# turboderp-org/exllamav2

Measured on NVIDIA H100. Metric: decode tokens/sec (bs=1) Llama2-7B EXL2-4.0bpw, higher is better.
Workload: dtype fp16 (int2-8 weights, fp32 accumulate)

## Files before the change

exllamav2_b200/csrc/attn_q4.cu:

```cuda
#include <algorithm>
#include <map>
#include <mutex>

#include "gemv_i8.cuh"
#include "kv_format.cuh"
#include "qmatrix.cuh"

namespace exl2b {

extern unsigned long long* g_dbg;
extern int g_dbg_cta, g_dbg_slot;

constexpr int AQ_THREADS = 256;
constexpr int AQ_WARPS = 8;
constexpr int AQ_MAX_QLEN = 8;

struct AttnQ4Params {
    const half* q;
    const half* k_new;
    const half* v_new;
    uint8_t* k_q;
    half* k_s;
    uint8_t* v_q;
    half* v_s;
    const int32_t* cache_seqlens;
    const int32_t* block_table;
    half* out;
    half* out_xp;
    const uint16_t* out_invperm;
    int q_len, H, KVH, hd, page_size, pages_per_seq, max_ctx;
    float scale_log2;
    const half* rope_sin;
    const half* rope_cos;
    int rope_neox, sincos_size;
    int out_plain;
    int32_t* err;
    int sc_len;
    int stage;
    int ring_slots;
    int batch;
    int busy_ctas;
    unsigned int* slot_cnt;
    int nsplit;
    float* ws;
    unsigned int* cnt;
    unsigned long long* dbg;
    int dbg_cta;
    int pass_len;
};
constexpr int AQ_SPLIT_MIN = 512;
constexpr int AQ_SUB = 128;
constexpr int AQ_RING = 4;
constexpr int AQ_STAGE = 512;
constexpr int AQ_SMEM_MAX = 200 * 1024;
constexpr int AQ_PASS_SMEM = 114 * 1024;
constexpr int AQ_PASS_MIN = 512;
constexpr int AQ_PASS_ALIGN = 256;
constexpr int AQ_QPAD = 36;
constexpr int AQ_QIB = 80;

__host__ __device__ constexpr int aq_sub(int kb, int vb) { return AQ_SUB * 4 / (kb > vb ? kb : vb); }

struct AttnSmem {
    uint32_t qrot, qi, qsum, qscl, red, wred, new_q, new_s, new_y, pages, sc, kst, vst, ksst, vsst, rq, rs, total;
};
__host__ __device__ inline AttnSmem attn_smem_map(int hd, int kb, int vb, int pages_per_seq, int sc_len, int stage, bool ring) {
    const uint32_t nsc = hd / 32, rowk = hd * kb / 8, rowv = hd * vb / 8, sub = aq_sub(kb, vb);
    AttnSmem m;
    m.qrot = 0;
    m.qi = m.qrot + nsc * AQ_QPAD * 4;
    m.qsum = m.qi + nsc * AQ_QIB;
    m.qscl = m.qsum + nsc * 4;
    m.red = m.qscl + nsc * 4;
    m.wred = m.red + AQ_WARPS * hd * 4;
    m.new_q = m.wred + 2 * AQ_WARPS * 4;
    m.new_s = m.new_q + AQ_MAX_QLEN * (rowk + rowv);
    m.new_y = m.new_s + 2 * AQ_MAX_QLEN * nsc * 2;
    m.pages = m.new_y + 2 * AQ_MAX_QLEN * hd * 4;
    m.sc = m.pages + ((pages_per_seq + 3) & ~3) * 4;
    m.kst = m.sc + ((sc_len + 3) & ~3) * 4;
    m.vst = m.kst + stage * rowk;
    m.ksst = m.vst + stage * rowv;
    m.vsst = m.ksst + stage * nsc * 2;
    m.rq = m.vsst + stage * nsc * 2;
    m.rs = m.rq + AQ_RING * sub * (rowk > rowv ? rowk : rowv);
    m.total = ring ? m.rs + AQ_RING * sub * nsc * 2 : m.rq;
    return m;
}

template <bool GLOBAL, typename T>
__device__ __forceinline__ T ld_rows(const T* p) {
    if constexpr (GLOBAL) return __ldg(p);
    else return *p;
}

template <int HD>
__device__ __forceinline__ half2 load_roped(const half* __restrict__ row, int un, int lane, const AttnQ4Params& P, int pos) {
    const half2 v = reinterpret_cast<const half2*>(row + un * 64)[lane];
    if (!P.rope_sin) return v;
    const half* sr = P.rope_sin + (size_t)pos * P.sincos_size;
    const half* cr = P.rope_cos + (size_t)pos * P.sincos_size;
    if (P.rope_neox) {
        half2 o;
        int col;
        bool first;
        if constexpr (HD == 128) {
            o = reinterpret_cast<const half2*>(row + (un ^ 1) * 64)[lane];
            col = 2 * lane;
            first = (un == 0);
        } else {
            o = __shfl_xor_sync(0xffffffffu, v, 16);
            col = 2 * (lane & 15);
            first = lane < 16;
        }
        const half2 c2 = *reinterpret_cast<const half2*>(cr + col);
        const half2 s2 = *reinterpret_cast<const half2*>(sr + col);
        if (first) return __hfma2(v, c2, __hmul2(o, __hneg2(s2)));
        return __hfma2(v, c2, __hmul2(o, s2));
    }
    const int col = un * 64 + 2 * lane;
    const half2 c01 = *reinterpret_cast<const half2*>(cr + col);
    half2 s01 = *reinterpret_cast<const half2*>(sr + col);
    uint32_t sb = *reinterpret_cast<uint32_t*>(&s01) ^ (1u << 15);
    s01 = *reinterpret_cast<half2*>(&sb);
    return __hfma2(__lowhigh2highlow(v), s01, __hmul2(v, c01));
}

__device__ __forceinline__ float nib_f(uint32_t n) { return __uint_as_float(0x4B000000u | n) - 8388616.0f; }
__device__ __forceinline__ float byte_f(uint32_t n) { return __uint_as_float(0x4B000000u | n) - 8388736.0f; }

__device__ __forceinline__ void cta_exit(const AttnQ4Params& P) {
    if (threadIdx.x == 0) slot_release(P.slot_cnt);
}

template <int HD, int KB, int VB>
struct AttnCta {
    static_assert((KB == 4 || KB == 8) && (VB == 4 || VB == 8), "element widths are 4 or 8 bits");
    static constexpr int ROWBK = HD * KB / 8;
    static constexpr int ROWBV = HD * VB / 8;
    static constexpr int ROWB = ROWBK > ROWBV ? ROWBK : ROWBV;
    static constexpr int SUB = aq_sub(KB, VB);
    static constexpr int NSC = HD / 32;
    static constexpr int VEC = HD / 32;
    static constexpr int UNITS = HD / 64;
    static constexpr int TPR = NSC, RPP = AQ_THREADS / TPR;
    static constexpr int KW = KB / 4;
    static constexpr uint32_t KFILL = KB == 4 ? 0x88888888u : 0x80808080u;

    const AttnQ4Params& P;
    float* qrot;
    uint8_t* qi;
    int* qsum;
    float* qscl;
    float* red;
    float* wred;
    uint8_t* new_q;
    half* new_s;
    float* new_y;
    int* pages_s;
    float* sc;
    uint8_t *kst, *vst;
    half *ksst, *vsst;
    uint8_t* rq;
    half* rs;
    int h, b, z, tid, warp, lane, group, kvh, kblk, krow;
    int seqlen, ns_act, p_lo, p_hi, c_hi, n_st, ntail;
    const int* bt;

    __device__ __forceinline__ AttnCta(const AttnQ4Params& P_, uint8_t* smem) : P(P_) {
        const AttnSmem m = attn_smem_map(HD, KB, VB, P.pages_per_seq, P.sc_len, P.stage, true);
        qrot = reinterpret_cast<float*>(smem + m.qrot);
        qi = smem + m.qi;
        qsum = reinterpret_cast<int*>(smem + m.qsum);
        qscl = reinterpret_cast<float*>(smem + m.qscl);
        red = reinterpret_cast<float*>(smem + m.red);
        wred = reinterpret_cast<float*>(smem + m.wred);
        new_q = smem + m.new_q;
        new_s = reinterpret_cast<half*>(smem + m.new_s);
        new_y = reinterpret_cast<float*>(smem + m.new_y);
        pages_s = reinterpret_cast<int*>(smem + m.pages);
        sc = reinterpret_cast<float*>(smem + m.sc);
        kst = smem + m.kst;
        vst = smem + m.vst;
        ksst = reinterpret_cast<half*>(smem + m.ksst);
        vsst = reinterpret_cast<half*>(smem + m.vsst);
        rq = smem + m.rq;
        rs = reinterpret_cast<half*>(smem + m.rs);
        h = (int)blockIdx.x % P.H;
        b = ((int)blockIdx.x / P.H) % P.batch;
        z = (int)blockIdx.x / (P.H * P.batch);
        tid = threadIdx.x;
        warp = tid >> 5;
        lane = tid & 31;
        group = P.H / P.KVH;
        kvh = h / group;
        kblk = tid & (TPR - 1);
        krow = tid / TPR;
    }

    __device__ __forceinline__ size_t row(int p) const {
        const int page = bt[p / P.page_size];
        return ((size_t)page * P.page_size + p % P.page_size) * P.KVH + kvh;
    }

    __device__ __forceinline__ bool prologue() {
        seqlen = P.cache_seqlens[b];
        if (seqlen < 0 || seqlen + P.q_len > P.max_ctx) {
            if (tid == 0 && P.err) atomicOr(P.err, 1);
            return false;
        }
        bt = P.block_table + (size_t)b * P.pages_per_seq;
        ns_act = 1;
        p_lo = 0;
        p_hi = seqlen + P.q_len;
        if (P.nsplit > 1) {
            const int n_all = seqlen + 1;
            ns_act = min(P.nsplit, max(1, (n_all + AQ_SPLIT_MIN - 1) / AQ_SPLIT_MIN));
            if (z >= ns_act) return false;
            const int chunk = (n_all + ns_act - 1) / ns_act;
            p_lo = z * chunk;
            p_hi = min(n_all, p_lo + chunk);
        }
        c_hi = min(p_hi, seqlen);
        n_st = max(0, min(c_hi - p_lo, P.stage));
        constexpr int CHK = ROWBK / 16, CHV = ROWBV / 16, CH = CHK > CHV ? CHK : CHV;
        for (int idx = tid; idx < n_st * CH; idx += AQ_THREADS) {
            const int pos = idx / CH, ch = idx - pos * CH;
            const size_t r = row(p_lo + pos);
            if (ch < CHK) cp_async16(smem_addr(kst + pos * ROWBK + ch * 16), P.k_q + r * ROWBK + ch * 16);
            if (ch < CHV) cp_async16(smem_addr(vst + pos * ROWBV + ch * 16), P.v_q + r * ROWBV + ch * 16);
        }
        for (int pos = tid; pos < n_st; pos += AQ_THREADS) {
            const size_t r = row(p_lo + pos);
            cp_async_small<NSC * 2>(smem_addr(ksst + pos * NSC), P.k_s + r * NSC);
            cp_async_small<NSC * 2>(smem_addr(vsst + pos * NSC), P.v_s + r * NSC);
        }
        asm volatile("cp.async.commit_group;" ::: "memory");
        for (int i = tid; i < P.pages_per_seq; i += AQ_THREADS) pages_s[i] = bt[i];
        bt = pages_s;
        ntail = ring_chunks();
        return true;
    }
    __device__ __forceinline__ int ring_chunks() const {
        return (P.ring_slots && c_hi > p_lo + n_st) ? (c_hi - (p_lo + n_st) + SUB - 1) / SUB : 0;
    }

    __device__ __forceinline__ void begin_pass(int lo, int hi, int nst) {
        p_lo = lo;
        c_hi = min(hi, seqlen);
        n_st = nst;
        ntail = ring_chunks();
    }

    __device__ __forceinline__ void rotate_q(int i, int un) {
        const half2 qh = load_roped<HD>(P.q + (((size_t)b * P.q_len + i) * P.H + h) * HD, un, lane, P, seqlen + i);
        float2 w = hadamard32_f(__half22float2(qh), lane);
        const float f = P.scale_log2 * (1.0f / 32.0f);
        const int e = un * 64 + 2 * lane;
        w.x *= f;
        w.y *= f;
        qrot[(e >> 5) * AQ_QPAD + (e & 31)] = w.x;
        qrot[(e >> 5) * AQ_QPAD + (e & 31) + 1] = w.y;
        float amax = fmaxf(fabsf(w.x), fabsf(w.y));
#pragma unroll
        for (int o = 1; o < 16; o <<= 1) amax = fmaxf(amax, __shfl_xor_sync(0xffffffffu, amax, o));
        const uint32_t ef = (__float_as_uint(amax * 1.000030518f) >> 23) & 0xffu;
        const float inv = amax > 0.f ? __uint_as_float((268u - ef) << 23) : 0.f;
        const uint32_t q0 = __float_as_uint(fmaf(w.x, inv, 12582912.f)), q1 = __float_as_uint(fmaf(w.y, inv, 12582912.f));
        int sum = (int)(q0 + q1 - 2u * 0x4B400000u);
#pragma unroll
        for (int o = 1; o < 16; o <<= 1) sum += __shfl_xor_sync(0xffffffffu, sum, o);
        const int blk = e >> 5, l16 = lane & 15;
        if constexpr (KB == 4) {
            const int j = l16 >> 2, m = l16 & 3;
            uint8_t* qb = qi + blk * AQ_QIB + j * 16 + m;
            qb[0] = (uint8_t)(q0 >> 8);
            qb[4] = (uint8_t)q0;
            qb[8] = (uint8_t)(q1 >> 8);
            qb[12] = (uint8_t)q1;
        } else {
            const int w8 = l16 >> 1;
            uint8_t* qb = qi + blk * AQ_QIB + (w8 >> 1) * 16 + (w8 & 1) * 8 + (l16 & 1) * 2;
            qb[0] = (uint8_t)(q0 >> 8);
            qb[1] = (uint8_t)(q1 >> 8);
            qb[4] = (uint8_t)q0;
            qb[5] = (uint8_t)q1;
        }
        if (l16 == 0) {
            qsum[blk] = sum;
            qscl[blk] = amax > 0.f ? __uint_as_float((ef - 14u) << 23) : 0.f;
        }
    }

    __device__ __forceinline__ void new_rows_and_first_query() {
        if (warp >= AQ_WARPS - UNITS) rotate_q(0, warp - (AQ_WARPS - UNITS));
        const int n_jobs = 2 * P.q_len * UNITS;
        for (int job = (warp >= AQ_WARPS - UNITS && n_jobs <= AQ_WARPS - UNITS) ? n_jobs : warp; job < n_jobs; job += AQ_WARPS) {
            const int kv = job / (P.q_len * UNITS), r = job - kv * P.q_len * UNITS;
            const int i = r / UNITS, un = r - i * UNITS;
            const half* src = (kv ? P.v_new : P.k_new) + (((size_t)b * P.q_len + i) * P.KVH + kvh) * HD;
            half2 w2 = kv ? reinterpret_cast<const half2*>(src + un * 64)[lane] : load_roped<HD>(src, un, lane, P, seqlen + i);
            {
                const float2 y = hadamard32_f(__half22float2(w2), lane);
                new_y[(kv * AQ_MAX_QLEN + i) * HD + un * 64 + 2 * lane] = y.x;
                new_y[(kv * AQ_MAX_QLEN + i) * HD + un * 64 + 2 * lane + 1] = y.y;
            }
            w2 = hadamard32_h(w2, lane);
            uint8_t* nq = new_q + (kv ? AQ_MAX_QLEN * ROWBK + i * ROWBV : i * ROWBK);
            half* ns = new_s + (kv * AQ_MAX_QLEN + i) * NSC + un * 2 + (lane >> 4);
            if ((kv ? VB : KB) == 4) {
                const KvCodes c = kv_quantise<4>(w2);
                nq[un * 32 + lane] = (uint8_t)(c.q0 | (c.q1 << 4));
                if ((lane & 15) == 0) *ns = c.scale;
            } else {
                const KvCodes c = kv_quantise<8>(w2);
                reinterpret_cast<uint16_t*>(nq + un * 64)[lane] = (uint16_t)(c.q0 | (c.q1 << 8));
                if ((lane & 15) == 0) *ns = c.scale;
            }
        }
    }

    template <int RB>
    __device__ __forceinline__ void ring_issue(int t, const uint8_t* gq, const half* gs) const {
        constexpr int CH = RB / 16;
        const int base = p_lo + n_st + t * SUB, cnt = min(SUB, c_hi - base), slot = t & (AQ_RING - 1);
        for (int idx = tid; idx < cnt * CH; idx += AQ_THREADS) {
            const int pos = idx / CH, ch = idx - pos * CH;
            cp_async16(smem_addr(rq + (slot * SUB + pos) * ROWB + ch * 16), gq + row(base + pos) * RB + ch * 16);
        }
        for (int pos = tid; pos < cnt; pos += AQ_THREADS)
            cp_async_small<NSC * 2>(smem_addr(rs + (slot * SUB + pos) * NSC), gs + row(base + pos) * NSC);
        asm volatile("cp.async.commit_group;" ::: "memory");
    }
    template <int RB, typename F>
    __device__ __forceinline__ void ring_pass(const uint8_t* gq, const half* gs, F&& consume) const {
        __syncthreads();
        for (int t = 0; t < AQ_RING; ++t) ring_issue<RB>(t, gq, gs);
        for (int t = 0; t < ntail; ++t) {
            asm volatile("cp.async.wait_group %0;" ::"n"(AQ_RING - 1) : "memory");
            __syncthreads();
            const int slot = t & (AQ_RING - 1);
            consume(p_lo + n_st + t * SUB, rq + slot * SUB * ROWB, rs + slot * SUB * NSC);
            __syncthreads();
            ring_issue<RB>(t + AQ_RING, gq, gs);
        }
    }

    struct KeyBlock {
        uint4 w[KW];
        uint32_t s;
    };
    __device__ __forceinline__ static KeyBlock key_none() {
        KeyBlock k;
#pragma unroll
        for (int u = 0; u < KW; ++u) k.w[u] = make_uint4(KFILL, KFILL, KFILL, KFILL);
        k.s = 0u;
        return k;
    }
    template <bool GLOBAL>
    __device__ __forceinline__ KeyBlock key_block(const uint8_t* rowq, const half* rows) const {
        KeyBlock k;
#pragma unroll
        for (int u = 0; u < KW; ++u) k.w[u] = ld_rows<GLOBAL>(reinterpret_cast<const uint4*>(rowq) + kblk * KW + u);
        k.s = ld_rows<GLOBAL>(reinterpret_cast<const unsigned short*>(rows) + kblk);
        return k;
    }
    __device__ __forceinline__ KeyBlock key_global(int p) const {
        const size_t r = row(p);
        return key_block<true>(P.k_q + r * ROWBK, P.k_s + r * NSC);
    }

    __device__ __forceinline__ float score_blk(const KeyBlock& k) const {
        const uint8_t* qb = qi + kblk * AQ_QIB;
        int v;
        if constexpr (KB == 4) {
            const uint32_t ww[4] = {k.w[0].x, k.w[0].y, k.w[0].z, k.w[0].w};
            int a0 = 0, a1 = 0, a2 = 0, a3 = 0;
#pragma unroll
            for (int j = 0; j < 4; ++j) {
                const uint4 qo = *reinterpret_cast<const uint4*>(qb + j * 16);
                const uint32_t lo = ww[j] & 0x0f0f0f0fu, hi = ww[j] & 0xf0f0f0f0u;
                a0 = dp4a_us(lo, qo.x, a0);
                a1 = dp4a_uu(lo, qo.y, a1);
                a2 = dp4a_us(hi, qo.z, a2);
                a3 = dp4a_uu(hi, qo.w, a3);
            }
            v = ((a0 << 8) + a1) + (((a2 << 8) + a3) >> 4) - 8 * qsum[kblk];
        } else {
            const uint32_t ww[8] = {k.w[0].x, k.w[0].y, k.w[0].z, k.w[0].w, k.w[1].x, k.w[1].y, k.w[1].z, k.w[1].w};
            int a0 = 0, a1 = 0, a2 = 0, a3 = 0;
#pragma unroll
            for (int j = 0; j < 4; ++j) {
                const uint4 qo = *reinterpret_cast<const uint4*>(qb + j * 16);
                a0 = dp4a_us(ww[2 * j], qo.x, a0);
                a1 = dp4a_uu(ww[2 * j], qo.y, a1);
                a2 = dp4a_us(ww[2 * j + 1], qo.z, a2);
                a3 = dp4a_uu(ww[2 * j + 1], qo.w, a3);
            }
            v = ((a0 + a2) << 8) + (a1 + a3) - 128 * qsum[kblk];
        }
        return __half2float(__ushort_as_half((unsigned short)k.s)) * qscl[kblk] * (float)v;
    }

    __device__ __forceinline__ void score_pos(int p, const KeyBlock& k, int n_ctx, float& lmax) const {
        float s = 0.f;
        if (p < n_ctx) {
            if (p >= seqlen) {
                const float4* y4 = reinterpret_cast<const float4*>(new_y + (p - seqlen) * HD + kblk * 32);
                const float4* q4 = reinterpret_cast<const float4*>(qrot + kblk * AQ_QPAD);
                float s0 = 0.f, s1 = 0.f, s2 = 0.f, s3 = 0.f;
#pragma unroll
                for (int j = 0; j < 8; ++j) {
                    const float4 a = q4[j], c = y4[j];
                    s0 = fmaf(a.x, c.x, s0);
                    s1 = fmaf(a.y, c.y, s1);
                    s2 = fmaf(a.z, c.z, s2);
                    s3 = fmaf(a.w, c.w, s3);
                }
                s = (s0 + s1) + (s2 + s3);
            } else {
                s = score_blk(k);
            }
        }
#pragma unroll
        for (int o = 1; o < TPR; o <<= 1) s += __shfl_xor_sync(0xffffffffu, s, o);
        if (p < n_ctx) {
            if (kblk == 0) sc[p - p_lo] = s;
            lmax = fmaxf(lmax, s);
        }
    }

    __device__ __forceinline__ float scores(int n_ctx) const {
        float lmax = -INFINITY;
        const int st_end = p_lo + n_st;
        int pb = p_lo;
        for (; pb < n_ctx && pb < st_end; pb += RPP) {
            const int pp = pb + krow;
            KeyBlock k = key_none();
            if (pp < st_end) k = key_block<false>(kst + (pp - p_lo) * ROWBK, ksst + (pp - p_lo) * NSC);
            else if (pp < min(n_ctx, seqlen)) k = key_global(pp);
            score_pos(pp, k, n_ctx, lmax);
        }
        if (ntail > 0) {
            ring_pass<ROWBK>(P.k_q, P.k_s, [&](int base, const uint8_t* rq_t, const half* rs_t) {
#pragma unroll 1
                for (int r0 = 0; r0 < SUB; r0 += RPP) {
                    if (base + r0 >= n_ctx) break;
                    const int rr = r0 + krow, pp = base + rr;
                    const bool in_sub = SUB >= RPP || rr < SUB;
                    KeyBlock k = key_none();
                    if (in_sub && pp < c_hi) k = key_block<false>(rq_t + rr * ROWB, rs_t + rr * NSC);
                    score_pos(in_sub ? pp : INT_MAX, k, n_ctx, lmax);
                }
            });
            pb = p_lo + n_st + ntail * SUB;
        }
        constexpr int TU = 2 / KW;
        for (; pb < n_ctx; pb += TU * RPP) {
            KeyBlock k[TU];
#pragma unroll
            for (int u = 0; u < TU; ++u) {
                const int pp = pb + u * RPP + krow;
                k[u] = key_none();
                if (pp < min(n_ctx, seqlen)) k[u] = key_global(pp);
            }
#pragma unroll
            for (int u = 0; u < TU; ++u)
                if (pb + u * RPP < n_ctx) score_pos(pb + u * RPP + krow, k[u], n_ctx, lmax);
        }
        return lmax;
    }

    __device__ __forceinline__ void softmax(float lmax, int n_ctx, float& mx, float& denom) const {
#pragma unroll
        for (int o = 16; o > 0; o >>= 1) lmax = fmaxf(lmax, __shfl_xor_sync(0xffffffffu, lmax, o));
        if (lane == 0) wred[warp] = lmax;
        __syncthreads();
        EXL2B_STAMP(P, 4);
        mx = wred[0];
#pragma unroll
        for (int w = 1; w < AQ_WARPS; ++w) mx = fmaxf(mx, wred[w]);
        float lsum = 0.f;
        for (int p = p_lo + tid; p < n_ctx; p += AQ_THREADS) {
            const float e = exp2f(sc[p - p_lo] - mx);
            sc[p - p_lo] = e;
            lsum += e;
        }
#pragma unroll
        for (int o = 16; o > 0; o >>= 1) lsum += __shfl_xor_sync(0xffffffffu, lsum, o);
        if (lane == 0) wred[AQ_WARPS + warp] = lsum;
        __syncthreads();
        denom = 0.f;
#pragma unroll
        for (int w = 0; w < AQ_WARPS; ++w) denom += wred[AQ_WARPS + w];
    }

    struct ValueRow {
        uint32_t x;
        uint32_t d;
    };
    __device__ __forceinline__ static ValueRow value_none() {
        if constexpr (VB == 4) return {0x8888u, 0u};
        else return {0u, 0x80808080u};
    }
    template <bool GLOBAL>
    __device__ __forceinline__ ValueRow value_row(const uint8_t* rowq, const half* rows) const {
        const uint32_t s = ld_rows<GLOBAL>(reinterpret_cast<const uint16_t*>(rows) + ((lane * VEC) >> 5));
        if constexpr (VB == 4) {
            uint32_t x;
            if constexpr (VEC == 4) x = ld_rows<GLOBAL>(reinterpret_cast<const uint16_t*>(rowq) + lane);
            else x = (uint32_t)ld_rows<GLOBAL>(rowq + lane) | 0x8800u;
            return {x | (s << 16), 0u};
        } else {
            if constexpr (VEC == 4) return {s, ld_rows<GLOBAL>(reinterpret_cast<const uint32_t*>(rowq) + lane)};
            else return {s, (uint32_t)ld_rows<GLOBAL>(reinterpret_cast<const uint16_t*>(rowq) + lane)};
        }
    }
    __device__ __forceinline__ void pv_fma(float (&acc)[VEC], const ValueRow& v, float pw) const {
        if constexpr (VB == 4) {
            const float pe = pw * __half2float(__ushort_as_half((unsigned short)(v.x >> 16)));
#pragma unroll
            for (int j = 0; j < VEC; ++j) acc[j] = fmaf(pe, nib_f((v.x >> (4 * j)) & 15u), acc[j]);
        } else {
            const float pe = pw * __half2float(__ushort_as_half((unsigned short)v.x));
#pragma unroll
            for (int j = 0; j < VEC; ++j) acc[j] = fmaf(pe, byte_f((v.d >> (8 * j)) & 0xffu), acc[j]);
        }
    }

    __device__ __forceinline__ void pv(int n_ctx) const {
        float acc[VEC];
#pragma unroll
        for (int j = 0; j < VEC; ++j) acc[j] = 0.f;
        const int st_end = p_lo + n_st;
#pragma unroll 4
        for (int p = p_lo + warp; p < st_end; p += AQ_WARPS) {
            const int r = p - p_lo;
            pv_fma(acc, value_row<false>(vst + r * ROWBV, vsst + r * NSC), sc[r]);
        }
        if (ntail > 0) {
            ring_pass<ROWBV>(P.v_q, P.v_s, [&](int base, const uint8_t* rq_t, const half* rs_t) {
#pragma unroll 4
                for (int r = warp; r < SUB; r += AQ_WARPS) {
                    const int pp = base + r;
                    if (pp < c_hi) pv_fma(acc, value_row<false>(rq_t + r * ROWB, rs_t + r * NSC), sc[pp - p_lo]);
                }
            });
        }
        for (int p0 = (ntail > 0 ? c_hi : st_end) + warp; p0 < c_hi; p0 += AQ_WARPS * 8) {
            ValueRow v[8];
#pragma unroll
            for (int u = 0; u < 8; ++u) {
                const int p = p0 + u * AQ_WARPS;
                v[u] = value_none();
                if (p < c_hi) {
                    const size_t r = row(p);
                    v[u] = value_row<true>(P.v_q + r * ROWBV, P.v_s + r * NSC);
                }
            }
#pragma unroll
            for (int u = 0; u < 8; ++u) {
                const int p = p0 + u * AQ_WARPS;
                if (p < c_hi) pv_fma(acc, v[u], sc[p - p_lo]);
            }
        }
        if (warp == 0) {
            for (int p = max(seqlen, p_lo); p < n_ctx; ++p) {
                const float pe = sc[p - p_lo];
                const float* y = new_y + (AQ_MAX_QLEN + p - seqlen) * HD + lane * VEC;
#pragma unroll
                for (int j = 0; j < VEC; ++j) acc[j] = fmaf(pe, y[j], acc[j]);
            }
        }
#pragma unroll
        for (int j = 0; j < VEC; ++j) red[warp * HD + lane * VEC + j] = acc[j];
    }

    __device__ __forceinline__ void append() const {
        constexpr int WK = ROWBK / 4, WV = ROWBV / 4;
        for (int idx = lane; idx < P.q_len * (WK + WV); idx += 32) {
            const int kv = idx >= P.q_len * WK, r = kv ? idx - P.q_len * WK : idx;
            const int ii = kv ? r / WV : r / WK, wd = kv ? r - ii * WV : r - ii * WK;
            const size_t rw = row(seqlen + ii);
            reinterpret_cast<uint32_t*>(kv ? P.v_q + rw * ROWBV : P.k_q + rw * ROWBK)[wd] =
                reinterpret_cast<const uint32_t*>(new_q + (kv ? AQ_MAX_QLEN * ROWBK + ii * ROWBV : ii * ROWBK))[wd];
        }
        for (int idx = lane; idx < 2 * P.q_len * NSC; idx += 32) {
            const int kv = idx / (P.q_len * NSC), r = idx - kv * P.q_len * NSC;
            const int ii = r / NSC, sidx = r - ii * NSC;
            (kv ? P.v_s : P.k_s)[row(seqlen + ii) * NSC + sidx] = new_s[(kv * AQ_MAX_QLEN + ii) * NSC + sidx];
        }
    }

    __device__ __forceinline__ float2 warp_sum() const {
        float2 w = make_float2(0.f, 0.f);
#pragma unroll
        for (int ww = 0; ww < AQ_WARPS; ++ww) {
            w.x += red[ww * HD + warp * 64 + 2 * lane];
            w.y += red[ww * HD + warp * 64 + 2 * lane + 1];
        }
        return w;
    }
    __device__ __forceinline__ void store_out(int i, float2 w, float L) const {
        w = hadamard32_f(w, lane);
        const float f = (1.0f / 32.0f) / L;
        const half2 o2 = __floats2half2_rn(w.x * f, w.y * f);
        reinterpret_cast<half2*>(P.out + (((size_t)b * P.q_len + i) * P.H + h) * HD + warp * 64)[lane] = o2;
        if (P.out_xp) {
            const int n = h * HD + warp * 64 + 2 * lane, m = b * P.q_len + i;
            const int k0 = P.out_invperm ? (int)P.out_invperm[n] : n, k1 = P.out_invperm ? (int)P.out_invperm[n + 1] : n + 1;
            if (P.out_plain) {
                P.out_xp[k0] = __low2half(o2);
                P.out_xp[k1] = __high2half(o2);
            } else {
                P.out_xp[(size_t)(k0 >> 3) * 64 + m * 8 + (k0 & 7)] = __low2half(o2);
                P.out_xp[(size_t)(k1 >> 3) * 64 + m * 8 + (k1 & 7)] = __high2half(o2);
            }
        }
    }
    __device__ __forceinline__ bool end_query(int i, float mx, float denom) const {
        return end_query(i, mx, denom, [&] { return warp_sum(); });
    }
    template <typename F>
    __device__ __forceinline__ bool end_query(int i, float mx, float denom, F&& out) const {
        if (ns_act > 1) {
            __shared__ int s_last;
            float* wsp = P.ws + (((size_t)b * P.H + h) * P.nsplit + z) * (HD + 2);
            if (warp < UNITS) __stcg(reinterpret_cast<float2*>(wsp + warp * 64) + lane, out());
            if (tid == 0) { __stcg(wsp + HD, mx); __stcg(wsp + HD + 1, denom); }
            __threadfence();
            __syncthreads();
            if (tid == 0) {
                const unsigned old = atomicAdd(P.cnt + (size_t)b * P.H + h, 1u);
                s_last = (old == (unsigned)ns_act - 1u);
                if (s_last) P.cnt[(size_t)b * P.H + h] = 0u;
                __threadfence();
            }
            __syncthreads();
            if (s_last && warp < UNITS) {
                const float* base = P.ws + ((size_t)b * P.H + h) * P.nsplit * (HD + 2);
                float M = -INFINITY;
                for (int sidx = 0; sidx < ns_act; ++sidx) M = fmaxf(M, __ldcg(base + (size_t)sidx * (HD + 2) + HD));
                float2 w = make_float2(0.f, 0.f);
                float L = 0.f;
                for (int sidx = 0; sidx < ns_act; ++sidx) {
                    const float* ps = base + (size_t)sidx * (HD + 2);
                    const float wgt = exp2f(__ldcg(ps + HD) - M);
                    const float2 a = __ldcg(reinterpret_cast<const float2*>(ps + warp * 64) + lane);
                    w.x = fmaf(wgt, a.x, w.x);
                    w.y = fmaf(wgt, a.y, w.y);
                    L = fmaf(wgt, __ldcg(ps + HD + 1), L);
                }
                store_out(i, w, L);
            }
            return false;
        }
        if (warp < UNITS) store_out(i, out(), denom);
        __syncthreads();
        return true;
    }
};

template <int HD, int KB, int VB>
__global__ void __launch_bounds__(AQ_THREADS, 2) attn_q4_kernel(const __grid_constant__ AttnQ4Params P) {
    extern __shared__ __align__(16) uint8_t smem[];
    EXL2B_STAMP(P, 0);
    griddep_launch_dependents();
    if ((int)blockIdx.x >= P.busy_ctas) {
        if (threadIdx.x == 0) slot_hold(P.slot_cnt, P.busy_ctas);
        return;
    }
    AttnCta<HD, KB, VB> c(P, smem);
    if (!c.prologue()) return cta_exit(P);
    EXL2B_STAMP(P, 1);
    griddep_wait();
    EXL2B_STAMP(P, 2);
    c.new_rows_and_first_query();
    asm volatile("cp.async.wait_group 0;" ::: "memory");
    __syncthreads();
    EXL2B_STAMP(P, 3);
    EXL2B_STAMP(P, 8);
    for (int i = 0; i < P.q_len; ++i) {
        const int n_ctx = (P.nsplit > 1) ? c.p_hi : c.seqlen + i + 1;
        if (i > 0) {
            if (c.warp < c.UNITS) c.rotate_q(i, c.warp);
            __syncthreads();
        }
        const float lmax = c.scores(n_ctx);
        EXL2B_STAMP(P, 9);
        float mx, denom;
        c.softmax(lmax, n_ctx, mx, denom);
        c.pv(n_ctx);
        __syncthreads();
        EXL2B_STAMP(P, 5);
        if (i == P.q_len - 1 && c.warp == AQ_WARPS - 1 && c.h % c.group == 0 && c.z == 0) c.append();
        if (!c.end_query(i, mx, denom)) return cta_exit(P);
    }
    if (P.dbg && threadIdx.x == 0) atomicMax(P.dbg + 7, globaltimer());
    cta_exit(P);
}

template <int HD, int KB, int VB>
__global__ void __launch_bounds__(AQ_THREADS, 2) attn_q4_passes_kernel(const __grid_constant__ AttnQ4Params P) {
    extern __shared__ __align__(16) uint8_t smem[];
    EXL2B_STAMP(P, 0);
    griddep_launch_dependents();
    if ((int)blockIdx.x >= P.busy_ctas) {
        if (threadIdx.x == 0) slot_hold(P.slot_cnt, P.busy_ctas);
        return;
    }
    AttnCta<HD, KB, VB> c(P, smem);
    if (!c.prologue()) return cta_exit(P);
    EXL2B_STAMP(P, 1);
    griddep_wait();
    EXL2B_STAMP(P, 2);
    c.new_rows_and_first_query();
    asm volatile("cp.async.wait_group 0;" ::: "memory");
    __syncthreads();
    EXL2B_STAMP(P, 3);
    float2* o = reinterpret_cast<float2*>(c.new_y + HD) + c.warp * 32 + c.lane;
    if (c.warp < c.UNITS) *o = make_float2(0.f, 0.f);
    float M = -INFINITY, L = 0.f;
    for (int pl = c.p_lo, nst = c.n_st; pl < c.p_hi; pl += P.pass_len, nst = 0) {
        const int ph = min(c.p_hi, pl + P.pass_len);
        c.begin_pass(pl, ph, nst);
        const float lmax = c.scores(ph);
        float mx, denom;
        c.softmax(lmax, ph, mx, denom);
        c.pv(ph);
        __syncthreads();
        const float mn = fmaxf(M, mx), a = exp2f(M - mn), w = exp2f(mx - mn);
        if (c.warp < c.UNITS) {
            const float2 s = c.warp_sum(), r = *o;
            *o = make_float2(fmaf(w, s.x, r.x * a), fmaf(w, s.y, r.y * a));
        }
        L = fmaf(w, denom, L * a);
        M = mn;
    }
    EXL2B_STAMP(P, 5);
    if (c.warp == AQ_WARPS - 1 && c.h % c.group == 0 && c.z == 0) c.append();
    if (!c.end_query(0, M, L, [&] { return *o; })) return cta_exit(P);
    if (P.dbg && threadIdx.x == 0) atomicMax(P.dbg + 7, globaltimer());
    cta_exit(P);
}

struct AttnLaunch {
    int nsplit;
    int sc_len;
    int ring_slots;
    int stage;
    int pass_len;
    AttnSmem smem;
};
static AttnLaunch attn_launch_plan(int kb, int vb, int hd, int q_len, int num_heads, int batch, int page_size, int pages_per_seq,
                                   int sms) {
    AttnLaunch L;
    const int max_ctx = page_size * pages_per_seq;
    L.nsplit = 1;
    if (q_len == 1 && max_ctx > 2 * AQ_SPLIT_MIN) {
        const int by_ctx = (max_ctx + AQ_SPLIT_MIN - 1) / AQ_SPLIT_MIN;
        const int by_sms = std::max(1, (2 * sms) / std::max(1, num_heads * batch));
        L.nsplit = std::max(1, std::min(std::min(by_ctx, by_sms), 16));
    }
    L.sc_len = L.nsplit > 1 ? std::max(AQ_SPLIT_MIN, (max_ctx + L.nsplit) / L.nsplit) + 8 : max_ctx + q_len;
    L.ring_slots = (max_ctx > 8192) ? AQ_RING : 0;
    const int rowk = hd * kb / 8, rowv = hd * vb / 8, nsc = hd / 32;
    const int window = L.ring_slots ? AQ_STAGE / 2 : AQ_STAGE;
    L.stage = (int)((size_t)window * (hd + 4 * nsc) / (size_t)(rowk + rowv + 4 * nsc)) / 64 * 64;
    L.smem = attn_smem_map(hd, kb, vb, pages_per_seq, L.sc_len, L.stage, L.ring_slots != 0);
    L.pass_len = 0;
    if (q_len == 1 && L.smem.total > (uint32_t)AQ_SMEM_MAX) {
        const uint32_t rest = attn_smem_map(hd, kb, vb, pages_per_seq, 0, L.stage, true).total;
        const int room = rest < (uint32_t)AQ_PASS_SMEM ? (int)((AQ_PASS_SMEM - rest) / 4) : 0;
        L.pass_len = std::max(AQ_PASS_MIN, room / AQ_PASS_ALIGN * AQ_PASS_ALIGN);
        L.sc_len = L.pass_len;
        L.smem = attn_smem_map(hd, kb, vb, pages_per_seq, L.sc_len, L.stage, true);
    }
    return L;
}

}

using namespace exl2b;

static int32_t* g_attn_err[64] = {nullptr};

namespace exl2b {
int attn_err_flag(int device, int32_t** flag) {
    if (!g_attn_err[device]) {
        EXL2B_CUDA(cudaMalloc(&g_attn_err[device], sizeof(int32_t)));
        EXL2B_CUDA(cudaMemset(g_attn_err[device], 0, sizeof(int32_t)));
    }
    *flag = g_attn_err[device];
    return 0;
}
}

struct AttnScratch {
    float* ws = nullptr;
    unsigned int* cnt = nullptr;
    size_t ws_floats = 0, n_cnt = 0;
};
static std::map<std::pair<int, cudaStream_t>, AttnScratch> g_attn_scratch;
static std::mutex g_attn_scratch_mutex;

static int attn_scratch(int device, cudaStream_t stream, int sms, AttnScratch** out) {
    std::lock_guard<std::mutex> lock(g_attn_scratch_mutex);
    AttnScratch& s = g_attn_scratch[{device, stream}];
    if (!s.ws) {
        const size_t floats = (size_t)2 * sms * (128 + 2), cnt = (size_t)sms;
        EXL2B_CUDA(cudaMalloc(&s.ws, floats * sizeof(float)));
        EXL2B_CUDA(cudaMalloc(&s.cnt, cnt * sizeof(unsigned int)));
        EXL2B_CUDA(cudaMemset(s.cnt, 0, cnt * sizeof(unsigned int)));
        EXL2B_CUDA(cudaDeviceSynchronize());
        s.ws_floats = floats;
        s.n_cnt = cnt;
    }
    *out = &s;
    return 0;
}

namespace exl2b {
int attn_scratch_query(int device, cudaStream_t stream, int kind, void** ptr, size_t* bytes) {
    std::lock_guard<std::mutex> lock(g_attn_scratch_mutex);
    const auto it = g_attn_scratch.find({device, stream});
    *ptr = nullptr;
    *bytes = 0;
    if (it == g_attn_scratch.end()) return 0;
    if (kind == EXL2B_SCRATCH_ATTN_WS) {
        *ptr = it->second.ws;
        *bytes = it->second.ws_floats * sizeof(float);
    } else {
        *ptr = it->second.cnt;
        *bytes = it->second.n_cnt * sizeof(unsigned int);
    }
    return 0;
}
}

extern "C" int exl2b_paged_attn_status(int device, int* status) {
    EXL2B_REQUIRE(status && device >= 0 && device < 64, "bad argument");
    *status = 0;
    if (!g_attn_err[device]) return 0;
    EXL2B_CUDA(cudaSetDevice(device));
    EXL2B_CUDA(cudaMemcpy(status, g_attn_err[device], sizeof(int), cudaMemcpyDeviceToHost));
    return 0;
}

extern "C" int exl2b_paged_attn_clear_status(int device) {
    EXL2B_REQUIRE(device >= 0 && device < 64, "bad argument");
    if (!g_attn_err[device]) return 0;
    EXL2B_CUDA(cudaSetDevice(device));
    EXL2B_CUDA(cudaMemset(g_attn_err[device], 0, sizeof(int)));
    return 0;
}

template <int KB, int VB>
static int attn_q_launch(int head_dim, dim3 grid, size_t smem, cudaStream_t stream, const AttnQ4Params& P) {
    if (P.pass_len) {
        if (head_dim == 128)
            EXL2B_CUDA(launch_pdl_f("attn", attn_q4_passes_kernel<128, KB, VB>, grid, dim3(AQ_THREADS), smem, stream, P));
        else
            EXL2B_CUDA(launch_pdl_f("attn", attn_q4_passes_kernel<64, KB, VB>, grid, dim3(AQ_THREADS), smem, stream, P));
        return 0;
    }
    if (head_dim == 128)
        EXL2B_CUDA(launch_pdl_f("attn", attn_q4_kernel<128, KB, VB>, grid, dim3(AQ_THREADS), smem, stream, P));
    else
        EXL2B_CUDA(launch_pdl_f("attn", attn_q4_kernel<64, KB, VB>, grid, dim3(AQ_THREADS), smem, stream, P));
    return 0;
}

template <int KB, int VB>
static int attn_q_set_smem() {
    EXL2B_CUDA(cudaFuncSetAttribute(attn_q4_kernel<128, KB, VB>, cudaFuncAttributeMaxDynamicSharedMemorySize, AQ_SMEM_MAX));
    EXL2B_CUDA(cudaFuncSetAttribute(attn_q4_kernel<64, KB, VB>, cudaFuncAttributeMaxDynamicSharedMemorySize, AQ_SMEM_MAX));
    EXL2B_CUDA(cudaFuncSetAttribute(attn_q4_passes_kernel<128, KB, VB>, cudaFuncAttributeMaxDynamicSharedMemorySize, AQ_SMEM_MAX));
    EXL2B_CUDA(cudaFuncSetAttribute(attn_q4_passes_kernel<64, KB, VB>, cudaFuncAttributeMaxDynamicSharedMemorySize, AQ_SMEM_MAX));
    return 0;
}

extern "C" int exl2b_paged_attn_decode_q(const uint16_t* q, const uint16_t* k_new, const uint16_t* v_new, uint8_t* k_cache,
                                         uint16_t* k_scales, uint8_t* v_cache, uint16_t* v_scales, const int32_t* cache_seqlens,
                                         const int32_t* block_table, uint16_t* out, int batch, int q_len, int num_heads,
                                         int num_kv_heads, int head_dim, int page_size, int pages_per_seq, float softmax_scale,
                                         exl2b_qmatrix_t out_consumer, const uint16_t* rope_sin, const uint16_t* rope_cos,
                                         int rope_style, int sincos_size, int wbits, exl2b_stream_t stream) {
    EXL2B_REQUIRE(q && k_new && v_new && k_cache && k_scales && v_cache && v_scales && cache_seqlens && block_table && out, "null argument");
    EXL2B_REQUIRE(wbits == 4 || wbits == 6 || wbits == 8, "cache wbits must be 4 (Q4), 6 (Q6) or 8 (Q8); got %d", wbits);
    const int kb = wbits == 4 ? 4 : 8, vb = wbits == 8 ? 8 : 4;
    EXL2B_REQUIRE(head_dim == 64 || head_dim == 128, "head_dim %d not supported (64 or 128)", head_dim);
    EXL2B_REQUIRE(num_heads % num_kv_heads == 0, "bad GQA ratio");
    EXL2B_REQUIRE(q_len >= 1 && q_len <= AQ_MAX_QLEN, "q_len %d outside the decode regime (1..%d)", q_len, AQ_MAX_QLEN);
    AttnQ4Params P = {};
    P.q = (const half*)q; P.k_new = (const half*)k_new; P.v_new = (const half*)v_new;
    P.k_q = k_cache; P.k_s = (half*)k_scales; P.v_q = v_cache; P.v_s = (half*)v_scales;
    P.cache_seqlens = cache_seqlens; P.block_table = block_table; P.out = (half*)out;
    P.q_len = q_len; P.H = num_heads; P.KVH = num_kv_heads; P.hd = head_dim;
    P.page_size = page_size; P.pages_per_seq = pages_per_seq;
    P.max_ctx = page_size * pages_per_seq;
    P.scale_log2 = softmax_scale * 1.4426950408889634f;
    if (out_consumer) {
        QMatrix* oc = (QMatrix*)out_consumer;
        EXL2B_REQUIRE(oc->v.layout == LAYOUT_TC && oc->v.K == num_heads * head_dim, "out_consumer does not take the attention output");
        EXL2B_REQUIRE(batch * q_len <= 8, "chained attention output needs at most 8 rows");
        int rc = qmatrix_chain_buffers(oc);
        if (rc) return rc;
        P.out_xp = oc->xp_buf;
        P.out_invperm = oc->invperm;
        P.out_plain = (batch * q_len == 1 && gemv_i8_enabled()) ? 1 : 0;
    }
    if (rope_style != 0 && rope_sin && rope_cos) {
        EXL2B_REQUIRE(sincos_size == head_dim, "fused RoPE needs sincos_size == head_dim (partial rotary: apply rope_ first)");
        P.rope_sin = (const half*)rope_sin;
        P.rope_cos = (const half*)rope_cos;
        P.rope_neox = rope_style == 2;
        P.sincos_size = sincos_size;
    }
    int dev = 0;
    EXL2B_CUDA(cudaGetDevice(&dev));
    EXL2B_REQUIRE(dev >= 0 && dev < 64, "bad device");
    const int sms = device_sm_count(dev);
    const AttnLaunch L = attn_launch_plan(kb, vb, head_dim, q_len, num_heads, batch, page_size, pages_per_seq, sms);
    if (L.pass_len)
        EXL2B_REQUIRE(L.smem.total <= AQ_SMEM_MAX,
                      "a page table of %d pages needs %u bytes of shared memory with passes of %d positions, above %d",
                      pages_per_seq, L.smem.total, L.pass_len, AQ_SMEM_MAX);
    EXL2B_REQUIRE(L.smem.total <= AQ_SMEM_MAX, "context of %d tokens does not fit the score buffer", P.max_ctx);
    {
        int rc = attn_err_flag(dev, &P.err);
        if (rc) return rc;
    }
    if (L.nsplit > 1) {
        AttnScratch* s = nullptr;
        int rc = attn_scratch(dev, (cudaStream_t)stream, sms, &s);
        if (rc) return rc;
        const size_t need = (size_t)batch * num_heads * L.nsplit * (head_dim + 2), need_c = (size_t)batch * num_heads;
        EXL2B_REQUIRE(need <= s->ws_floats && need_c <= s->n_cnt,
                      "split-KV launch needs %zu floats / %zu counters, above the per-stream bound %zu / %zu", need, need_c,
                      s->ws_floats, s->n_cnt);
        P.ws = s->ws;
        P.cnt = s->cnt;
    }
    P.nsplit = L.nsplit;
    P.sc_len = L.sc_len;
    P.ring_slots = L.ring_slots;
    P.stage = L.stage;
    P.pass_len = L.pass_len;
    P.dbg = exl2b::g_dbg ? exl2b::g_dbg + 32 * (exl2b::g_dbg_slot++ % 64) : nullptr;
    P.dbg_cta = 0;
    static bool attr_set[64] = {false};
    if (!attr_set[dev]) {
        int rc = attn_q_set_smem<4, 4>();
        if (!rc) rc = attn_q_set_smem<8, 4>();
        if (!rc) rc = attn_q_set_smem<8, 8>();
        if (rc) return rc;
        attr_set[dev] = true;
    }
    static SlotCounters slot_cnts;
    int rc = next_slot_counter(slot_cnts, dev, &P.slot_cnt);
    if (rc) return rc;
    P.batch = batch;
    P.busy_ctas = num_heads * batch * L.nsplit;
    dim3 grid(slot_holders_disabled() ? P.busy_ctas : std::max(P.busy_ctas, sms));
    if (wbits == 4) return attn_q_launch<4, 4>(head_dim, grid, L.smem.total, (cudaStream_t)stream, P);
    if (wbits == 6) return attn_q_launch<8, 4>(head_dim, grid, L.smem.total, (cudaStream_t)stream, P);
    return attn_q_launch<8, 8>(head_dim, grid, L.smem.total, (cudaStream_t)stream, P);
}
```

Before: 483.7.

## Add fused single-pass online-softmax attention path for fully staged decode

When q_len is 1 and every key/value row is already staged in shared memory, each warp now handles a contiguous slice of positions. It computes scores, an online softmax and the PV accumulation in one pass, then the warps merge their partial results, replacing the separate scores, softmax and PV phases and the barriers between them. RoPE sin/cos loads and an L2 prefetch of the output inverse permutation are moved before the grid-dependency wait so they overlap the previous kernel. A trailing barrier after the last query is dropped. The change adds a second code path that must match the original numerically. The round loop structure also looks unusual, and end_query is called with a new signature that is not shown.

```diff
diff --git a/exllamav2_b200/csrc/attn_q4.cu b/exllamav2_b200/csrc/attn_q4.cu
--- a/exllamav2_b200/csrc/attn_q4.cu
+++ b/exllamav2_b200/csrc/attn_q4.cu
@@ -94,36 +94,37 @@
     else return *p;
 }
 
+struct RopeCs {
+    half2 c, s;
+};
 template <int HD>
-__device__ __forceinline__ half2 load_roped(const half* __restrict__ row, int un, int lane, const AttnQ4Params& P, int pos) {
+__device__ __forceinline__ RopeCs rope_cs(int un, int lane, const AttnQ4Params& P, int pos) {
+    const int col = !P.rope_neox ? un * 64 + 2 * lane : HD == 128 ? 2 * lane : 2 * (lane & 15);
+    return {*reinterpret_cast<const half2*>(P.rope_cos + (size_t)pos * P.sincos_size + col),
+            *reinterpret_cast<const half2*>(P.rope_sin + (size_t)pos * P.sincos_size + col)};
+}
+
+template <int HD>
+__device__ __forceinline__ half2 load_roped(const half* __restrict__ row, int un, int lane, const AttnQ4Params& P, const RopeCs& cs) {
     const half2 v = reinterpret_cast<const half2*>(row + un * 64)[lane];
     if (!P.rope_sin) return v;
-    const half* sr = P.rope_sin + (size_t)pos * P.sincos_size;
-    const half* cr = P.rope_cos + (size_t)pos * P.sincos_size;
     if (P.rope_neox) {
         half2 o;
-        int col;
         bool first;
         if constexpr (HD == 128) {
             o = reinterpret_cast<const half2*>(row + (un ^ 1) * 64)[lane];
-            col = 2 * lane;
             first = (un == 0);
         } else {
             o = __shfl_xor_sync(0xffffffffu, v, 16);
-            col = 2 * (lane & 15);
             first = lane < 16;
         }
-        const half2 c2 = *reinterpret_cast<const half2*>(cr + col);
-        const half2 s2 = *reinterpret_cast<const half2*>(sr + col);
-        if (first) return __hfma2(v, c2, __hmul2(o, __hneg2(s2)));
-        return __hfma2(v, c2, __hmul2(o, s2));
-    }
-    const int col = un * 64 + 2 * lane;
-    const half2 c01 = *reinterpret_cast<const half2*>(cr + col);
-    half2 s01 = *reinterpret_cast<const half2*>(sr + col);
+        if (first) return __hfma2(v, cs.c, __hmul2(o, __hneg2(cs.s)));
+        return __hfma2(v, cs.c, __hmul2(o, cs.s));
+    }
+    half2 s01 = cs.s;
     uint32_t sb = *reinterpret_cast<uint32_t*>(&s01) ^ (1u << 15);
     s01 = *reinterpret_cast<half2*>(&sb);
-    return __hfma2(__lowhigh2highlow(v), s01, __hmul2(v, c01));
+    return __hfma2(__lowhigh2highlow(v), s01, __hmul2(v, cs.c));
 }
 
 __device__ __forceinline__ float nib_f(uint32_t n) { return __uint_as_float(0x4B000000u | n) - 8388616.0f; }
@@ -166,6 +167,7 @@
     int h, b, z, tid, warp, lane, group, kvh, kblk, krow;
     int seqlen, ns_act, p_lo, p_hi, c_hi, n_st, ntail;
     const int* bt;
+    RopeCs cs0;
 
     __device__ __forceinline__ AttnCta(const AttnQ4Params& P_, uint8_t* smem) : P(P_) {
         const AttnSmem m = attn_smem_map(HD, KB, VB, P.pages_per_seq, P.sc_len, P.stage, true);
@@ -241,6 +243,18 @@
         ntail = ring_chunks();
         return true;
     }
+    __device__ __forceinline__ void load_static() {
+        cs0 = P.rope_sin ? rope_cs<HD>(rope_unit(), lane, P, seqlen) : RopeCs{};
+        if (P.out_invperm && warp < UNITS && lane == 0)
+            asm volatile("prefetch.global.L2 [%0];" ::"l"(P.out_invperm + h * HD + warp * 64));
+    }
+    __device__ __forceinline__ int rope_unit() const {
+        return warp >= AQ_WARPS - UNITS ? warp - (AQ_WARPS - UNITS) : warp % UNITS;
+    }
+    __device__ __forceinline__ half2 roped(const half* row, int un, int i) const {
+        const bool pre = !P.rope_sin || (i == 0 && un == rope_unit());
+        return load_roped<HD>(row, un, lane, P, pre ? cs0 : rope_cs<HD>(un, lane, P, seqlen + i));
+    }
     __device__ __forceinline__ int ring_chunks() const {
         return (P.ring_slots && c_hi > p_lo + n_st) ? (c_hi - (p_lo + n_st) + SUB - 1) / SUB : 0;
     }
@@ -253,7 +267,7 @@
     }
 
     __device__ __forceinline__ void rotate_q(int i, int un) {
-        const half2 qh = load_roped<HD>(P.q + (((size_t)b * P.q_len + i) * P.H + h) * HD, un, lane, P, seqlen + i);
+        const half2 qh = roped(P.q + (((size_t)b * P.q_len + i) * P.H + h) * HD, un, i);
         float2 w = hadamard32_f(__half22float2(qh), lane);
         const float f = P.scale_log2 * (1.0f / 32.0f);
         const int e = un * 64 + 2 * lane;
@@ -299,7 +313,7 @@
             const int kv = job / (P.q_len * UNITS), r = job - kv * P.q_len * UNITS;
             const int i = r / UNITS, un = r - i * UNITS;
             const half* src = (kv ? P.v_new : P.k_new) + (((size_t)b * P.q_len + i) * P.KVH + kvh) * HD;
-            half2 w2 = kv ? reinterpret_cast<const half2*>(src + un * 64)[lane] : load_roped<HD>(src, un, lane, P, seqlen + i);
+            half2 w2 = kv ? reinterpret_cast<const half2*>(src + un * 64)[lane] : roped(src, un, i);
             {
                 const float2 y = hadamard32_f(__half22float2(w2), lane);
                 new_y[(kv * AQ_MAX_QLEN + i) * HD + un * 64 + 2 * lane] = y.x;
@@ -402,26 +416,24 @@
         return __half2float(__ushort_as_half((unsigned short)k.s)) * qscl[kblk] * (float)v;
     }
 
+    __device__ __forceinline__ float score_new(int i) const {
+        const float4* y4 = reinterpret_cast<const float4*>(new_y + i * HD + kblk * 32);
+        const float4* q4 = reinterpret_cast<const float4*>(qrot + kblk * AQ_QPAD);
+        float s0 = 0.f, s1 = 0.f, s2 = 0.f, s3 = 0.f;
+#pragma unroll
+        for (int j = 0; j < 8; ++j) {
+            const float4 a = q4[j], c = y4[j];
+            s0 = fmaf(a.x, c.x, s0);
+            s1 = fmaf(a.y, c.y, s1);
+            s2 = fmaf(a.z, c.z, s2);
+            s3 = fmaf(a.w, c.w, s3);
+        }
+        return (s0 + s1) + (s2 + s3);
+    }
+
     __device__ __forceinline__ void score_pos(int p, const KeyBlock& k, int n_ctx, float& lmax) const {
         float s = 0.f;
-        if (p < n_ctx) {
-            if (p >= seqlen) {
-                const float4* y4 = reinterpret_cast<const float4*>(new_y + (p - seqlen) * HD + kblk * 32);
-                const float4* q4 = reinterpret_cast<const float4*>(qrot + kblk * AQ_QPAD);
-                float s0 = 0.f, s1 = 0.f, s2 = 0.f, s3 = 0.f;
-#pragma unroll
-                for (int j = 0; j < 8; ++j) {
-                    const float4 a = q4[j], c = y4[j];
-                    s0 = fmaf(a.x, c.x, s0);
-                    s1 = fmaf(a.y, c.y, s1);
-                    s2 = fmaf(a.z, c.z, s2);
-                    s3 = fmaf(a.w, c.w, s3);
-                }
-                s = (s0 + s1) + (s2 + s3);
-            } else {
-                s = score_blk(k);
-            }
-        }
+        if (p < n_ctx) s = p >= seqlen ? score_new(p - seqlen) : score_blk(k);
 #pragma unroll
         for (int o = 1; o < TPR; o <<= 1) s += __shfl_xor_sync(0xffffffffu, s, o);
         if (p < n_ctx) {
@@ -574,6 +586,72 @@
         }
 #pragma unroll
         for (int j = 0; j < VEC; ++j) red[warp * HD + lane * VEC + j] = acc[j];
+    }
+
+    __device__ __forceinline__ bool all_staged() const { return P.q_len == 1 && ntail == 0 && c_hi - p_lo <= n_st; }
+    __device__ __forceinline__ void staged_pass(float& M, float& L, float2& w) const {
+        constexpr int G = 32 / TPR;
+        const int per = (p_hi - p_lo + AQ_WARPS * G - 1) / (AQ_WARPS * G) * G;
+        const int lo = p_lo + warp * per, hi = min(p_hi, lo + per), c_end = min(hi, seqlen);
+        const float* y_new = new_y + AQ_MAX_QLEN * HD + lane * VEC;
+        float m = -INFINITY, l = 0.f, acc[VEC];
+#pragma unroll
+        for (int j = 0; j < VEC; ++j) acc[j] = 0.f;
+        for (int pb = lo; pb < hi; pb += G) {
+            const int pp = pb + lane / TPR;
+            float s = 0.f;
+            if (pp < c_end) s = score_blk(key_block<false>(kst + (pp - p_lo) * ROWBK, ksst + (pp - p_lo) * NSC));
+            else if (pp < hi) s = score_new(0);
+#pragma unroll
+            for (int o = 1; o < TPR; o <<= 1) s += __shfl_xor_sync(0xffffffffu, s, o);
+            if (pp >= hi) s = -INFINITY;
+            float mn = s;
+#pragma unroll
+            for (int o = TPR; o < 32; o <<= 1) mn = fmaxf(mn, __shfl_xor_sync(0xffffffffu, mn, o));
+            mn = fmaxf(m, mn);
+            const float a = exp2f(m - mn), e = exp2f(s - mn);
+            m = mn;
+            l = fmaf(l, a, kblk == 0 ? e : 0.f);
+#pragma unroll
+            for (int j = 0; j < VEC; ++j) acc[j] *= a;
+#pragma unroll 2
+            for (int r = 0; r < G; ++r) {
+                const int p = pb + r;
+                const float pw = __shfl_sync(0xffffffffu, e, r * TPR);
+                if (p < c_end) {
+                    pv_fma(acc, value_row<false>(vst + (p - p_lo) * ROWBV, vsst + (p - p_lo) * NSC), pw);
+                } else if (p < hi) {
+#pragma unroll
+                    for (int j = 0; j < VEC; ++j) acc[j] = fmaf(pw, y_new[j], acc[j]);
+                }
+            }
+        }
+#pragma unroll
+        for (int o = TPR; o < 32; o <<= 1) l += __shfl_xor_sync(0xffffffffu, l, o);
+#pragma unroll
+        for (int j = 0; j < VEC; ++j) red[warp * HD + lane * VEC + j] = acc[j];
+        if (lane == 0) {
+            wred[warp] = m;
+            wred[AQ_WARPS + warp] = l;
+        }
+        EXL2B_STAMP(P, 4);
+        __syncthreads();
+        EXL2B_STAMP(P, 5);
+        M = -INFINITY;
+        L = 0.f;
+        w = make_float2(0.f, 0.f);
+        if (warp < UNITS) {
+#pragma unroll
+            for (int ww = 0; ww < AQ_WARPS; ++ww) M = fmaxf(M, wred[ww]);
+#pragma unroll
+            for (int ww = 0; ww < AQ_WARPS; ++ww) {
+                const float wgt = exp2f(wred[ww] - M);
+                const float2 a = reinterpret_cast<const float2*>(red + ww * HD + warp * 64)[lane];
+                w.x = fmaf(wgt, a.x, w.x);
+                w.y = fmaf(wgt, a.y, w.y);
+                L = fmaf(wgt, wred[AQ_WARPS + ww], L);
+            }
+        }
     }
 
     __device__ __forceinline__ void append() const {
@@ -656,7 +734,7 @@
             return false;
         }
         if (warp < UNITS) store_out(i, out(), denom);
-        __syncthreads();
+        if (i + 1 < P.q_len) __syncthreads();
         return true;
     }
 };
@@ -673,28 +751,45 @@
     AttnCta<HD, KB, VB> c(P, smem);
     if (!c.prologue()) return cta_exit(P);
     EXL2B_STAMP(P, 1);
-    griddep_wait();
-    EXL2B_STAMP(P, 2);
-    c.new_rows_and_first_query();
-    asm volatile("cp.async.wait_group 0;" ::: "memory");
-    __syncthreads();
-    EXL2B_STAMP(P, 3);
-    EXL2B_STAMP(P, 8);
-    for (int i = 0; i < P.q_len; ++i) {
-        const int n_ctx = (P.nsplit > 1) ? c.p_hi : c.seqlen + i + 1;
-        if (i > 0) {
-            if (c.warp < c.UNITS) c.rotate_q(i, c.warp);
+    const auto after_wait = [&] {
+        c.load_static();
+        griddep_wait();
+        EXL2B_STAMP(P, 2);
+        c.new_rows_and_first_query();
+        asm volatile("cp.async.wait_group 0;" ::: "memory");
+        __syncthreads();
+        EXL2B_STAMP(P, 3);
+        EXL2B_STAMP(P, 8);
+    };
+    if (c.all_staged()) {
+        float M = 0.f, L = 0.f;
+        float2 w = make_float2(0.f, 0.f);
+#pragma unroll 1
+        for (int round = HD == 128 ? 0 : 1; round < 2; ++round) {
+            if (round == 1) after_wait();
+            c.staged_pass(M, L, w);
+        }
+        if (P.dbg && threadIdx.x == 0) atomicAdd(P.dbg + 10, 1ull);
+        if (c.warp == AQ_WARPS - 1 && c.h % c.group == 0 && c.z == 0) c.append();
+        if (!c.end_query(0, M, L, [&] { return w; })) return cta_exit(P);
+    } else {
+        after_wait();
+        for (int i = 0; i < P.q_len; ++i) {
+            const int n_ctx = (P.nsplit > 1) ? c.p_hi : c.seqlen + i + 1;
+            if (i > 0) {
+                if (c.warp < c.UNITS) c.rotate_q(i, c.warp);
+                __syncthreads();
+            }
+            const float lmax = c.scores(n_ctx);
+            EXL2B_STAMP(P, 9);
+            float mx, denom;
+            c.softmax(lmax, n_ctx, mx, denom);
+            c.pv(n_ctx);
             __syncthreads();
-        }
-        const float lmax = c.scores(n_ctx);
-        EXL2B_STAMP(P, 9);
-        float mx, denom;
-        c.softmax(lmax, n_ctx, mx, denom);
-        c.pv(n_ctx);
-        __syncthreads();
-        EXL2B_STAMP(P, 5);
-        if (i == P.q_len - 1 && c.warp == AQ_WARPS - 1 && c.h % c.group == 0 && c.z == 0) c.append();
-        if (!c.end_query(i, mx, denom)) return cta_exit(P);
+            EXL2B_STAMP(P, 5);
+            if (i == P.q_len - 1 && c.warp == AQ_WARPS - 1 && c.h % c.group == 0 && c.z == 0) c.append();
+            if (!c.end_query(i, mx, denom)) return cta_exit(P);
+        }
     }
     if (P.dbg && threadIdx.x == 0) atomicMax(P.dbg + 7, globaltimer());
     cta_exit(P);
@@ -712,6 +807,7 @@
     AttnCta<HD, KB, VB> c(P, smem);
     if (!c.prologue()) return cta_exit(P);
     EXL2B_STAMP(P, 1);
+    c.load_static();
     griddep_wait();
     EXL2B_STAMP(P, 2);
     c.new_rows_and_first_query();
```

Result: faster. 505.4 (median of 6 runs) (+4.5%).
